# jaehyuck0103/OpenMAVIS

Hardware: AMD Instinct MI355X
Metric: multi-cam frames/sec (ORB extract+match) + LocalBA iters/sec, 5x720x540 (higher is better)
Workload: dtype u8

## Files before the change

### include/omv.h

```cpp
#ifndef OMV_H
#define OMV_H

#include <stddef.h>
#include <stdint.h>

#ifdef __cplusplus
extern "C" {
#endif

typedef int omv_status;
#define OMV_OK 0
#define OMV_ERR_ARG 1
#define OMV_ERR_HIP 2
#define OMV_ERR_CAPACITY 3
#define OMV_ERR_NO_DEVICE 4

typedef struct omv_orb_params {
    int nfeatures;
    float scale_factor;
    int nlevels;
    int ini_th_fast;
    int min_th_fast;
} omv_orb_params;

// ... 38 lines not shown
    float min_x, max_x;
    float min_y, max_y;
    int nlevels;
    float scale_factors[16];
    int cam_model[8];
} omv_frame_geom;

typedef struct omv_mp_view {
    const uint8_t *desc;
    const float *proj_x;
    const float *proj_y;
    const float *view_cos;
    const int32_t *level;
    const uint8_t *in_view;
    const float *track_depth;
    const uint8_t *is_bad;
    const uint8_t *has_obs;
} omv_mp_view;

typedef struct omv_matcher omv_matcher;

omv_status omv_matcher_create(int max_frames, int n_cams, int kp_cap, int max_mps, omv_matcher **out);
omv_status omv_matcher_destroy(omv_matcher *m);

omv_status omv_matcher_assign_grid(omv_matcher *m, int n_frames, const omv_frame_geom *geom, const omv_kp *kps,
                                   const int *n_kp, void *stream);
omv_status omv_matcher_grid_debug(omv_matcher *m, int frame, int cam, int32_t *cell_start, int32_t *idx);

omv_status omv_matcher_search_projection(omv_matcher *m, int n_frames, const omv_frame_geom *geom, const omv_kp *kps,
                                         const uint8_t *desc, const int *n_kp, const omv_mp_view *mps, int M, float th,
                                         int far_points, float th_far, float nnratio, const int32_t *l2r,
                                         const int32_t *r2l, const uint8_t *kp_occ_init, int32_t *kp_to_mp,
                                         int *n_matches, void *stream);

omv_status omv_matcher_stereo_lapping(omv_matcher *m, int n_frames, const uint8_t *desc, const int *n_kp,
                                      const int *mono, double ratio, int32_t *l2r, int32_t *r2l, void *stream);

omv_status omv_matcher_stereo_triangulate(omv_matcher *m, int n_frames, int n_cams, int kp_cap, const omv_kp *kps,
                                          const int *n_kp, const int *mono, const float *cams, const float *Rlr,
                                          const float *tlr, const float *level_sigma2, int nlevels, int32_t *l2r,
                                          int32_t *r2l, float *depth, float *p3d, void *stream);

omv_status omv_matcher_last_error(omv_matcher *m);

omv_status omv_matcher_enable_timing(omv_matcher *m, int on);
omv_status omv_matcher_stage_ms(omv_matcher *m, double *ms4, int reset);

omv_status omv_bf_knn2(int n_pairs, const uint8_t *query, int q_cap, const int *nq, const uint8_t *train, int t_cap,
                       const int *nt, int32_t *idx2, int32_t *dist2, void *stream);
int omv_bf_knn2_path(int n_pairs, int q_cap, int t_cap);

typedef struct omv_se3f {
    float q[4];
    float t[3];
} omv_se3f;

typedef struct omv_last_frame {
    const float *pos;
    const uint8_t *desc;
    const uint8_t *valid;
    const uint8_t *has_obs;
    const omv_kp *kps;
    int S;
} omv_last_frame;

omv_status omv_matcher_search_last_frame(omv_matcher *m, int n_frames, const omv_frame_geom *geom, const omv_kp *kps,
// ... 600 lines not shown
```

### openmavis_amd/_lib.py

```python
import ctypes
import os

_HERE = os.path.dirname(os.path.abspath(__file__))
LIB_PATH = os.path.join(_HERE, "libomv_hip.so")

OMV_OK = 0
OMV_ERR_ARG = 1
OMV_ERR_HIP = 2
OMV_ERR_CAPACITY = 3
OMV_ERR_NO_DEVICE = 4
CAM_KB8 = 0
CAM_PINHOLE = 1
_ERRS = {1: "bad argument", 2: "HIP runtime error", 3: "device capacity exceeded", 4: "no HIP device"}


class OmvError(RuntimeError):
    pass


def check(status, what="omv call"):
    if status != OMV_OK:
        raise OmvError(f"{what} failed: {_ERRS.get(status, status)} ({status})")


# ... 202 lines not shown
                ("trials", ctypes.c_int), ("lambda_", ctypes.c_double), ("lambda_init", ctypes.c_double),
                ("mono_chi2", ctypes.c_void_p), ("mono_outlier", ctypes.c_void_p),
                ("stereo_chi2", ctypes.c_void_p), ("stereo_outlier", ctypes.c_void_p)]


try:
    import numpy as _np

    KP_DTYPE = _np.dtype([("x", "<f4"), ("y", "<f4"), ("size", "<f4"), ("angle", "<f4"),
                          ("response", "<f4"), ("octave", "<i4")])
except ImportError:
    KP_DTYPE = None

_VP, _I, _F, _SZ = ctypes.c_void_p, ctypes.c_int, ctypes.c_float, ctypes.c_size_t
ALLREDUCE_FN = ctypes.CFUNCTYPE(ctypes.c_int, ctypes.c_void_p, ctypes.c_void_p, ctypes.c_size_t, ctypes.c_void_p)
SIGNATURES = {
    "omv_orb_create": (_I, [ctypes.POINTER(OrbParams), _I, _I, _I, ctypes.POINTER(_VP)]),
    "omv_orb_destroy": (_I, [_VP]),
    "omv_selftest_node_sort": (_I, [_VP, _VP, _I, _VP, _VP]),
    "omv_orb_max_keypoints": (_I, [_VP]),
    "omv_orb_scale_tables": (_I, [_VP, _VP, _VP, _VP, _VP]),
    "omv_orb_extract_batch": (_I, [_VP, _I, _VP, _SZ, _SZ, _VP, _VP, _VP, _VP, _VP, _VP]),
    "omv_orb_extract_host": (_I, [_VP, _VP, _SZ, _I, _I, _VP, _VP, _VP, _VP]),
    "omv_orb_last_error": (_I, [_VP]),
    "omv_orb_enable_timing": (_I, [_VP, _I]),
    "omv_orb_set_harris": (_I, [_VP, _VP]),
    "omv_orb_stage_ms": (_I, [_VP, _VP, ctypes.POINTER(ctypes.c_longlong), _I]),
    "omv_orb_last_counts": (_I, [_VP, ctypes.POINTER(ctypes.c_longlong), ctypes.POINTER(ctypes.c_longlong)]),
    "omv_orb_debug_level": (_I, [_VP, _I, _I, _VP, ctypes.POINTER(_I), ctypes.POINTER(_I)]),
    "omv_matcher_create": (_I, [_I, _I, _I, _I, ctypes.POINTER(_VP)]),
    "omv_matcher_destroy": (_I, [_VP]),
    "omv_matcher_assign_grid": (_I, [_VP, _I, ctypes.POINTER(FrameGeom), _VP, _VP, _VP]),
    "omv_matcher_grid_debug": (_I, [_VP, _I, _I, _VP, _VP]),
    "omv_matcher_enable_timing": (_I, [_VP, _I]),
    "omv_matcher_last_error": (_I, [_VP]),
    "omv_matcher_stage_ms": (_I, [_VP, _VP, _I]),
    "omv_matcher_search_projection": (_I, [_VP, _I, ctypes.POINTER(FrameGeom), _VP, _VP, _VP,
                                           ctypes.POINTER(MpView), _I, _F, _I, _F, _F, _VP, _VP, _VP, _VP,
                                           _VP, _VP]),
    "omv_matcher_stereo_lapping": (_I, [_VP, _I, _VP, _VP, _VP, ctypes.c_double, _VP, _VP, _VP]),
    "omv_bf_knn2": (_I, [_I, _VP, _I, _VP, _VP, _I, _VP, _VP, _VP, _VP]),
    "omv_bf_knn2_path": (_I, [_I, _I, _I]),
    "omv_matcher_search_last_frame": (_I, [_VP, _I, ctypes.POINTER(FrameGeom), _VP, _VP, _VP, _VP, _VP, _VP,
                                           ctypes.POINTER(SE3f), ctypes.POINTER(LastFrame), _F, _I, _F, _I, _VP, _VP,
                                           _VP, _VP]),
    "omv_frustum": (_I, [_I, _VP, ctypes.POINTER(Rig), ctypes.POINTER(MpWorld), _I, _F, ctypes.POINTER(MpTrack), _VP,
                         _VP]),
    "omv_lba_create": (_I, [_I, _I, _I, _I, _I, ctypes.POINTER(_VP)]),
    "omv_lba_destroy": (_I, [_VP]),
    "omv_lba_set_problem": (_I, [_VP, ctypes.POINTER(LbaProblem)]),
    "omv_lba_optimize": (_I, [_VP, ctypes.POINTER(LbaOpts), ctypes.POINTER(LbaProblem), ctypes.POINTER(LbaResult)]),
    "omv_lba_evaluate": (_I, [_VP, _VP, _VP, _VP, _VP]),
    "omv_lba_evaluate_stereo": (_I, [_VP, _VP, _VP, _VP]),
    "omv_lba_stage_ms": (_I, [_VP, _VP, ctypes.POINTER(_I)]),
    "omv_lba_host_syncs": (_I, [_VP, ctypes.POINTER(_I), ctypes.POINTER(_I)]),
    "omv_lba_enable_timing": (_I, [_VP, _I]),
    "omv_lba_set_driver": (_I, [_VP, _I]),
    "omv_lba_reset": (_I, [_VP]),
    "omv_lba_set_comm": (_I, [_VP, _I, _I, _VP, _VP]),
    "omv_tri_debug": (_I, [_VP, _VP, _VP, _VP, _VP, _VP, _F, _F, _VP]),
    "omv_matcher_stereo_triangulate": (_I, [_VP, _I, _I, _I, _VP, _VP, _VP, _VP, _VP, _VP, _VP, _I, _VP, _VP, _VP,
                                            _VP, _VP]),
    "omv_matcher_search_for_triangulation": (_I, [_VP, _I, ctypes.POINTER(TriPair), _VP, _VP, _I, _I, _I, _VP, _VP]),
    "omv_matcher_search_by_bow": (_I, [_VP, _I, ctypes.POINTER(BowJob), _I, _F, _I, _VP, _VP]),
    "omv_matcher_bow_rescans": (_I, [ctypes.POINTER(ctypes.c_int64), _I]),
    "omv_matcher_search_for_initialization": (_I, [_VP, _I, _VP, ctypes.POINTER(FrameGeom), _VP, _VP, _VP, _VP, _I,
# ... 124 lines not shown
```

### openmavis_amd/csrc/match.hip

```cpp
#include <hip/hip_runtime.h>

#include <climits>
#include <cstdlib>
#include <cstring>
#include <type_traits>
#include <cmath>
#include <cstdio>
#include <vector>

#include "../../include/omv.h"
#include "omv_camera.h"
#include "omv_device.h"
#include "omv_host.h"

namespace {

using omv::kGridCols, omv::kGridRows;
constexpr int kCells = omv::kGridCells;
constexpr int kTH_HIGH = 100;
constexpr int kTop = 16;
constexpr int kMaxCams = 8;
constexpr size_t kResolveLds = 150 * 1024;

struct FrameArgs {
// ... 140 lines not shown
    int count;
    __device__ __forceinline__ void reset() { key[0] = key[1] = ~0ull, count = 0; }
    __device__ __forceinline__ void insert_at(int idx, int dist, int oct, int q) {
        const uint64_t k = ((uint64_t)dist << 40) | ((uint64_t)q << 20) | ((uint64_t)oct << 16) | (uint64_t)idx;
        key[1] = k < key[0] ? key[0] : (k < key[1] ? k : key[1]);
        key[0] = k < key[0] ? k : key[0];
    }
};
__device__ __forceinline__ uint32_t key_rec(uint64_t k) {
    return (uint32_t)(k & 0xffff) | ((uint32_t)(k >> 40) << 16) | ((uint32_t)((k >> 16) & 0xf) << 25);
}

struct TopSeq {
    uint32_t key[kTop];
    int n, count;
    __device__ __forceinline__ void reset() {
#pragma unroll
        for (int q = 0; q < kTop; ++q) key[q] = ~0u;
        n = count = 0;
    }
    __device__ __forceinline__ void insert(int idx, int dist, int oct) {
        const uint32_t k = ((uint32_t)dist << 23) | ((uint32_t)oct << 16) | (uint32_t)idx;
        const uint32_t kk = k | 0x7fffffu;
#pragma unroll
        for (int q = kTop - 1; q > 0; --q) key[q] = kk < key[q - 1] ? key[q - 1] : (kk < key[q] ? k : key[q]);
        key[0] = kk < key[0] ? k : key[0];
        n = min(n + 1, kTop);
    }
    __device__ __forceinline__ int idx(int q) const { return (int)(key[q] & 0xffff); }
    __device__ __forceinline__ int oct(int q) const { return (int)((key[q] >> 16) & 0x7f); }
    __device__ __forceinline__ int dist(int q) const { return (int)(key[q] >> 23); }
    __device__ __forceinline__ uint32_t rec(int q) const {
        return (uint32_t)idx(q) | ((uint32_t)dist(q) << 16) | ((uint32_t)oct(q) << 25);
    }
};

template <class Blocked, class TopT>
__device__ void scan_window(const FrameArgs &f, int frame, int cam, float x, float y, float r, int minL, int maxL,
                            const uint64_t dmp[4], Blocked blocked, TopT &t) {
    t.reset();
    omv::GridRange w;
    OMV_GRID_WINDOW_OR(x, y, r, f.min_x, f.min_y, f.invW, f.invH, w, return)
    const bool checkLevels = (minL > 0) || (maxL >= 0);
    const size_t fc = (size_t)frame * f.n_cams + cam;
    const int32_t *cs = f.cell_start + fc * (kCells + 1);
    const int32_t *ci = f.cell_idx + fc * f.kp_cap;
    const omv_kp *kp = f.kps + fc * f.kp_cap;
    const uint8_t *dd = f.desc + fc * f.kp_cap * 32;
    for (int ix = w.x0; ix <= w.x1; ++ix) {
        const int c0 = ix * kGridRows + w.y0, c1 = ix * kGridRows + w.y1;
        const int e = cs[c1 + 1];
        int p = cs[c0];
        int inext = p < e ? ci[p] : 0;
        for (; p < e; ++p) {
            const int i = inext;
            if (p + 1 < e) inext = ci[p + 1];
            const omv_kp k = kp[i];
            uint64_t d[4];
            omv::load_desc(dd + (size_t)i * 32, d);
            if (checkLevels) {
                if (k.octave < minL) continue;
                if (maxL >= 0 && k.octave > maxL) continue;
            }
            if (!(fabsf(k.x - x) < r && fabsf(k.y - y) < r)) continue;
            if (blocked(cam * f.kp_cap + i)) continue;
            ++t.count;
// ... 135 lines not shown
    const int g = lane % G;
    for (int q0 = 0; q0 < nq; q0 += 64 / G) {
        if (q0 + lane / G >= nq) break;
        const long long gid = g0 + queue[wave][q0 + lane / G];
        const int c = (int)(gid % C);
        const long long fm = gid / C;
        const int frame = (int)(fm / m.M);
        const size_t bc = (size_t)gid;
        std::conditional_t<G == 1, TopSeq, Top> t;
        t.reset();
        uint64_t dmp[4];
        omv::load_desc(m.desc + (size_t)fm * 32, dmp);
        const float r = window_radius(f, m, bc, c, th, th != 1.0f);
        const uint8_t *occ = occ_init ? occ_init + (size_t)frame * C * f.kp_cap : nullptr;
        if constexpr (G == 1) {
            scan_window(f, frame, c, m.proj_x[bc], m.proj_y[bc], r, m.level[bc] - 1, m.level[bc], dmp,
                        [&](int slot) { return occ && occ[slot]; }, t);
        } else {
            scan_window_coop<G>(f, frame, c, m.proj_x[bc], m.proj_y[bc], r, m.level[bc] - 1, m.level[bc], dmp,
                                [&](int slot) { return occ && occ[slot]; }, t, g);
            merge_top<G>(t);
        }
        if (g == 0) store_record(&recs[bc], t);
    }
}

constexpr int kStageThreads = 512;
constexpr uint32_t kStageBlocked = 1u << 31;
constexpr size_t kStageLdsMax = 80 * 1024;
constexpr int kScanGroup = 4;
constexpr int kStageUnroll = 3;
constexpr int kStageMaxIt = 4;
constexpr int kStageBuckets = 32;

__host__ __device__ inline size_t stage_lds_bytes(int kp_cap, int pw) {
    return (size_t)kp_cap * (32 + 8 + 4) + (size_t)(kCells + 1) * 4 + (size_t)(kStageThreads / 64) * pw * 4;
}

__device__ __forceinline__ void scan_window_lds(const FrameArgs &f, float x, float y, float r, int minL, int maxL,
                                                const uint64_t dmp[4], const int *scs, const float2 *sxy,
                                                const uint32_t *smeta, const uint4 *sdesc, TopSeq &t) {
    t.reset();
    omv::GridRange w;
    OMV_GRID_WINDOW_OR(x, y, r, f.min_x, f.min_y, f.invW, f.invH, w, return)
    const bool checkLevels = (minL > 0) || (maxL >= 0);
    for (int ix = w.x0; ix <= w.x1; ++ix) {
        const int e = scs[ix * kGridRows + w.y1 + 1];
        for (int p0 = scs[ix * kGridRows + w.y0]; p0 < e; p0 += kScanGroup) {
            float2 k[kScanGroup];
            uint32_t meta[kScanGroup];
#pragma unroll
            for (int u = 0; u < kScanGroup; ++u) k[u] = sxy[p0 + u], meta[u] = smeta[p0 + u];
#pragma unroll
            for (int u = 0; u < kScanGroup; ++u) {
                const int oct = (int)((meta[u] >> 16) & 0x7f);
                bool ok = p0 + u < e;
                if (checkLevels) ok = ok && oct >= minL && !(maxL >= 0 && oct > maxL);
                ok = ok && fabsf(k[u].x - x) < r && fabsf(k[u].y - y) < r && !(meta[u] & kStageBlocked);
                if (!ok) continue;
                const int p = p0 + u;
                const uint4 a = sdesc[2 * p], b = sdesc[2 * p + 1];
                const uint64_t d[4] = {(uint64_t)a.x | ((uint64_t)a.y << 32), (uint64_t)a.z | ((uint64_t)a.w << 32),
                                       (uint64_t)b.x | ((uint64_t)b.y << 32), (uint64_t)b.z | ((uint64_t)b.w << 32)};
                ++t.count;
                t.insert((int)(meta[u] & 0xffff), omv::hamming256(dmp, d), oct);
            }
        }
    }
}

__global__ void __launch_bounds__(kStageThreads) cand_stage_kernel(FrameArgs f, MpArgs m, int n_frames, float th,
                                                                   const uint8_t *occ_init, Rec *recs, int *counts,
                                                                   int *flags, int far_points, float th_far,
                                                                   int n_chunks, int pw, int n_blocks) {
    extern __shared__ __align__(16) unsigned char stage_lds[];
    const int C = f.n_cams, cap = f.kp_cap, M = m.M;
    const int blk = omv::xcd_block(n_blocks);
    if (blk < 0) return;
    const int chunk = blk % n_chunks, fc = blk / n_chunks, cam = fc % C, frame = fc / C;
    uint4 *sdesc = reinterpret_cast<uint4 *>(stage_lds);
    float2 *sxy = reinterpret_cast<float2 *>(stage_lds + (size_t)cap * 32);
    uint32_t *smeta = reinterpret_cast<uint32_t *>(stage_lds + (size_t)cap * 40);
    int *scs = reinterpret_cast<int *>(stage_lds + (size_t)cap * 44);
    int *queue = scs + kCells + 1;
    __shared__ int bucket[kStageBuckets + 1];
    const int tid = threadIdx.x, wave = tid >> 6, lane = tid & 63;
    if (tid <= kStageBuckets) bucket[tid] = 0;
    __syncthreads();
    const int32_t *cs = f.cell_start + (size_t)fc * (kCells + 1);
    const int32_t *ci = f.cell_idx + (size_t)fc * cap;
    const omv_kp *kp = f.kps + (size_t)fc * cap;
    const uint4 *dd = reinterpret_cast<const uint4 *>(f.desc + (size_t)fc * cap * 32);
    const uint8_t *occ = occ_init ? occ_init + ((size_t)frame * C + cam) * cap : nullptr;
    const int n_in = cs[kCells];
    for (int c = tid; c <= kCells; c += kStageThreads) scs[c] = cs[c];
    int idx[kStageUnroll];
#pragma unroll
    for (int u = 0; u < kStageUnroll; ++u) {
        const int p = u * kStageThreads + tid;
        idx[u] = p < n_in ? ci[p] : -1;
    }
    const int p0 = chunk * (kStageThreads / 64) * pw;
    int key[kStageMaxIt], lv[kStageMaxIt];
    bool iv[kStageMaxIt];
    float vc[kStageMaxIt];
#pragma unroll
    for (int it = 0; it < kStageMaxIt; ++it) {
        const int i = p0 + wave * pw + it * 64 + lane;
        const bool valid = it * 64 + lane < pw && i < M;
        const size_t bc = ((size_t)frame * M + (valid ? i : 0)) * C + cam;
        iv[it] = valid && m.in_view[bc];
        lv[it] = valid ? m.level[bc] : -1;
        vc[it] = valid ? m.view_cos[bc] : 0.0f;
    }
#pragma unroll
    for (int it = 0; it < kStageMaxIt; ++it) {
        key[it] = -1;
        const int i = p0 + wave * pw + it * 64 + lane;
        if (it * 64 + lane >= pw || i >= M) continue;
        const size_t fm = (size_t)frame * M + i, bc = fm * C + cam;
        if (cam == 0) {
            flags[fm] = point_flags(m, f, fm, frame, i, C, far_points, th_far);
        }
        if (iv[it] && lv[it] >= 0 && lv[it] < f.nlevels) {
            key[it] = 2 * lv[it] + (vc[it] > 0.998 ? 0 : 1);
            atomicAdd(&bucket[key[it]], 1);
        }
    }
    for (int s0 = 0; s0 < n_in; s0 += kStageThreads * kStageUnroll) {
        if (s0 > 0) {
#pragma unroll
            for (int u = 0; u < kStageUnroll; ++u) {
                const int p = s0 + u * kStageThreads + tid;
                idx[u] = p < n_in ? ci[p] : -1;
            }
        }
        float x[kStageUnroll], y[kStageUnroll];
        int oct[kStageUnroll];
        uint4 da[kStageUnroll], db[kStageUnroll];
        bool bl[kStageUnroll];
#pragma unroll
        for (int u = 0; u < kStageUnroll; ++u) {
            const int i = max(idx[u], 0);
            x[u] = kp[i].x, y[u] = kp[i].y, oct[u] = kp[i].octave;
            da[u] = dd[2 * i], db[u] = dd[2 * i + 1];
            bl[u] = occ && occ[i];
        }
#pragma unroll
        for (int u = 0; u < kStageUnroll; ++u) {
            const int p = s0 + u * kStageThreads + tid;
            if (idx[u] < 0) continue;
            sxy[p] = make_float2(x[u], y[u]);
            smeta[p] = (uint32_t)idx[u] | ((uint32_t)(oct[u] & 0x7f) << 16) | (bl[u] ? kStageBlocked : 0u);
            sdesc[2 * p] = da[u], sdesc[2 * p + 1] = db[u];
        }
    }
    __syncthreads();
    if (tid < 64) {
        const int c = tid < kStageBuckets ? bucket[tid] : 0;
        const int incl = omv::wave_incl_scan_i32(c, lane);
        if (tid < kStageBuckets) bucket[tid] = incl - c;
        if (tid == kStageBuckets - 1) bucket[kStageBuckets] = incl;
    }
    __syncthreads();
#pragma unroll
    for (int it = 0; it < kStageMaxIt; ++it)
        if (key[it] >= 0) queue[atomicAdd(&bucket[key[it]], 1)] = wave * pw + it * 64 + lane;
    __syncthreads();
    const int nq = bucket[kStageBuckets];
    for (int q = wave * 64 + lane; q - lane < nq; q += kStageThreads) {
        if (q >= nq) break;
        const int i = p0 + queue[q];
        const size_t fm = (size_t)frame * M + i, bc = fm * C + cam;
        TopSeq t;
        uint64_t dmp[4];
        omv::load_desc(m.desc + fm * 32, dmp);
        const float r = window_radius(f, m, bc, cam, th, th != 1.0f);
        scan_window_lds(f, m.proj_x[bc], m.proj_y[bc], r, m.level[bc] - 1, m.level[bc], dmp, scs, sxy, smeta, sdesc, t);
        store_record(&recs[bc], t);
    }
}

constexpr int kMaxRevived = 64;
constexpr int kMaxDomains = kMaxCams - 1;
constexpr int kListCap = 128;

struct ResolveArgs {
    FrameArgs f;
    MpArgs m;
    const Rec *recs;
    const int *counts;
    const int *flags;
    const int32_t *l2r, *r2l;
    const uint8_t *occ_init;
    int32_t *kp_to_mp;
    int *n_matches;
    int *err;
    float th, th_far, nnratio;
    int far_points;
    int lds_k2m;
};


__device__ __forceinline__ bool bit_of(const uint32_t *bits, int s) { return (bits[s >> 5] >> (s & 31)) & 1u; }

__device__ bool in_window(const FrameArgs &f, int frame, int c, int slot, float x, float y, float r, int lvl) {
    const omv_kp k = f.kps[((size_t)frame * f.n_cams) * f.kp_cap + slot];
    const int px = (int)roundf((k.x - f.min_x) * f.invW), py = (int)roundf((k.y - f.min_y) * f.invH);
    if (px < 0 || px >= kGridCols || py < 0 || py >= kGridRows) return false;
    const int x0 = max(0, (int)floorf((x - f.min_x - r) * f.invW));
    const int x1 = min(kGridCols - 1, (int)ceilf((x - f.min_x + r) * f.invW));
    const int y0 = max(0, (int)floorf((y - f.min_y - r) * f.invH));
    const int y1 = min(kGridRows - 1, (int)ceilf((y - f.min_y + r) * f.invH));
// ... 1572 lines not shown
omv_status omv_frustum(int n_frames, const omv_frame_pose *poses, const omv_rig *rig, const omv_mp_world *mp, int M,
                       float viewing_cos_limit, const omv_mp_track *out, int32_t *n_in_view, void *stream) {
    if (n_frames <= 0 || !poses || !rig || !mp || !out || M < 0 || rig->n_cams <= 0 || rig->n_cams > kMaxCams ||
        rig->n_levels <= 0 || !cam_models_ok(rig->model, rig->n_cams))
        return OMV_ERR_ARG;
    if (M == 0) return OMV_OK;
    hipStream_t st = (hipStream_t)stream;
    frustum_kernel<<<dim3((M + 255) / 256, n_frames), 256, 0, st>>>(poses, *rig, *mp, M, viewing_cos_limit, *out,
                                                                    n_in_view);
    HIP_OK(hipGetLastError());
    return OMV_OK;
}

omv_status omv_matcher_create(int max_frames, int n_cams, int kp_cap, int max_mps, omv_matcher **out) {
    if (!out || max_frames <= 0 || n_cams <= 0 || n_cams > kMaxCams || kp_cap <= 0 || kp_cap > 65535 || max_mps < 0)
        return OMV_ERR_ARG;
    if (resolve_lds_bytes(n_cams, kp_cap, max_mps) > kResolveLds - kResolveStaticLds || lf_resolve_lds_bytes(n_cams, kp_cap) > kResolveLds)
        return OMV_ERR_ARG;
    int ndev = 0;
    if (hipGetDeviceCount(&ndev) != hipSuccess || ndev == 0) return OMV_ERR_NO_DEVICE;
    const int resolve_dyn = (int)(kResolveLds - kResolveStaticLds);
    HIP_OK(hipFuncSetAttribute((const void *)resolve_kernel<true>, hipFuncAttributeMaxDynamicSharedMemorySize, resolve_dyn));
    HIP_OK(hipFuncSetAttribute((const void *)resolve_kernel<false>, hipFuncAttributeMaxDynamicSharedMemorySize, resolve_dyn));
    HIP_OK(hipFuncSetAttribute((const void *)lf_resolve_kernel, hipFuncAttributeMaxDynamicSharedMemorySize, (int)kResolveLds));
    HIP_OK(hipFuncSetAttribute((const void *)cand_stage_kernel, hipFuncAttributeMaxDynamicSharedMemorySize, (int)kStageLdsMax));
    auto h = std::make_unique<omv_matcher>();
    h->max_frames = max_frames, h->n_cams = n_cams, h->kp_cap = kp_cap, h->max_mps = max_mps;
    if (const char *e = getenv("OMV_BOW_TOP")) h->knobs.bow_top = atoi(e);
    if (const char *e = getenv("OMV_TRI_SLICES")) h->knobs.tri_slices = atoi(e);
    if (const char *e = getenv("OMV_TRI_ECAP")) h->knobs.tri_ecap = atoi(e);
    if (const char *e = getenv("OMV_TRI_WALK")) h->knobs.tri_walk_seq = strcmp(e, "seq") == 0 ? 1 : 0;
    if (const char *e = getenv("OMV_CAND")) h->knobs.cand_mode = strcmp(e, "global") == 0 ? 1 : strcmp(e, "lds") == 0 ? 2 : 0;
    if (const char *e = getenv("OMV_CAND_PW")) h->knobs.cand_pw = atoi(e);
    h->knobs.knn_mode = knn_mode_env(), h->knobs.knn_idx_limit = knn_idx_limit_env();
    const size_t fc = (size_t)max_frames * n_cams;
    const size_t knn = (size_t)2 * max_frames * kp_cap;
    omv::DeviceArena &mem = h->mem;
    if (!mem.alloc(&h->d_cell_start, fc * (kCells + 1)) || !mem.alloc(&h->d_cell_idx, fc * kp_cap) ||
        !mem.alloc(&h->d_recs, fc * max_mps) || !mem.alloc(&h->d_counts, fc * max_mps) ||
        !mem.alloc(&h->d_flags, (size_t)max_frames * max_mps) || !mem.alloc(&h->d_knn_i, knn) ||
        !mem.alloc(&h->d_knn_d, knn) || !mem.alloc(&h->d_err, 1))
        return OMV_ERR_HIP;
    HIP_OK(hipMemset(h->d_err, 0, sizeof(int)));
    *out = h.release();
    return OMV_OK;
}

omv_status omv_matcher_enable_timing(omv_matcher *h, int on) {
    if (!h) return OMV_ERR_ARG;
    h->timing = on != 0;
    return OMV_OK;
}

omv_status omv_matcher_stage_ms(omv_matcher *h, double *ms4, int reset) {
    if (!h || !ms4) return OMV_ERR_ARG;
    HIP_OK(hipStreamSynchronize(h->last));
    for (auto &p : h->ev) {
        float ms = 0.f;
        (void)hipEventElapsedTime(&ms, p.second.first, p.second.second);
        h->stage_ms[p.first] += ms;
        (void)hipEventDestroy(p.second.first);
        (void)hipEventDestroy(p.second.second);
    }
    h->ev.clear();
    for (int k = 0; k < 4; ++k) ms4[k] = h->stage_ms[k];
    if (reset)
// ... 9 lines not shown
    HIP_OK(hipMemset(h->d_err, 0, sizeof(int)));
    return e;
}

omv_status omv_matcher_destroy(omv_matcher *h) {
    if (!h) return OMV_ERR_ARG;
    delete h;
    return OMV_OK;
}

omv_status omv_matcher_assign_grid(omv_matcher *h, int n_frames, const omv_frame_geom *g, const omv_kp *kps,
                                   const int *n_kp, void *stream) {
    if (!h || !g || !kps || !n_kp || n_frames <= 0 || n_frames > h->max_frames || g->n_cams != h->n_cams)
        return OMV_ERR_ARG;
    FrameArgs f;
    if (!cam_models_ok(g->cam_model, h->n_cams)) return OMV_ERR_ARG;
    fill_frame(h, g, kps, nullptr, n_kp, f);
    hipStream_t st = (hipStream_t)stream;
    h->last = st;
    hipEvent_t e0 = h->timing ? mk_event(st) : nullptr;
    grid_kernel<<<n_frames * h->n_cams, 256, 0, st>>>(f, h->d_cell_start, h->d_cell_idx);
    if (h->timing) h->ev.push_back({0, {e0, mk_event(st)}});
    HIP_OK(hipGetLastError());
    return OMV_OK;
}

omv_status omv_matcher_grid_debug(omv_matcher *h, int frame, int cam, int32_t *cell_start, int32_t *idx) {
    if (!h || frame < 0 || frame >= h->max_frames || cam < 0 || cam >= h->n_cams) return OMV_ERR_ARG;
    HIP_OK(hipStreamSynchronize(h->last));
    const size_t fc = (size_t)frame * h->n_cams + cam;
    HIP_OK(hipMemcpy(cell_start, h->d_cell_start + fc * (kCells + 1), sizeof(int32_t) * (kCells + 1),
                     hipMemcpyDeviceToHost));
    HIP_OK(hipMemcpy(idx, h->d_cell_idx + fc * h->kp_cap, sizeof(int32_t) * h->kp_cap, hipMemcpyDeviceToHost));
    return OMV_OK;
}

omv_status omv_matcher_search_projection(omv_matcher *h, int n_frames, const omv_frame_geom *g, const omv_kp *kps,
                                         const uint8_t *desc, const int *n_kp, const omv_mp_view *mps, int M, float th,
                                         int far_points, float th_far, float nnratio, const int32_t *l2r,
                                         const int32_t *r2l, const uint8_t *kp_occ_init, int32_t *kp_to_mp,
                                         int *n_matches, void *stream) {
    if (!h || !g || !kps || !desc || !n_kp || !mps || !kp_to_mp || !n_matches || n_frames <= 0 ||
        n_frames > h->max_frames || M < 0 || M > h->max_mps || g->n_cams != h->n_cams)
        return OMV_ERR_ARG;
    if (h->n_cams > 1 && (!l2r || !r2l)) return OMV_ERR_ARG;
    hipStream_t st = (hipStream_t)stream;
    h->last = st;
    FrameArgs f;
    if (!cam_models_ok(g->cam_model, h->n_cams)) return OMV_ERR_ARG;
    fill_frame(h, g, kps, desc, n_kp, f);
    MpArgs m{mps->desc, mps->proj_x, mps->proj_y, mps->view_cos, mps->level, mps->in_view, mps->track_depth,
             mps->is_bad, mps->has_obs, M};
    hipEvent_t e0 = h->timing ? mk_event(st) : nullptr;
    if (M > 0) {
        const long long tot = (long long)n_frames * M * h->n_cams;
        int pw = 128;
        while (pw > 16 && (long long)n_frames * h->n_cams * ((M + 8 * pw - 1) / (8 * pw)) < 1024) pw >>= 1;
        if (h->knobs.cand_pw > 0) pw = min(h->knobs.cand_pw, 64 * kStageMaxIt);
        const bool staged = h->knobs.cand_mode == 2 || (h->knobs.cand_mode == 0 && tot > 262144);
        if (staged && stage_lds_bytes(h->kp_cap, pw) <= kStageLdsMax) {
            const int n_chunks = (M + 8 * pw - 1) / (8 * pw);
            const int nb = n_frames * h->n_cams * n_chunks;
            cand_stage_kernel<<<omv::xcd_grid(nb), kStageThreads, stage_lds_bytes(h->kp_cap, pw), st>>>(
                f, m, n_frames, th, kp_occ_init, h->d_recs, h->d_counts, h->d_flags, far_points, th_far, n_chunks, pw, nb);
        } else if (tot <= 65536) {
            const int nb = (int)((tot + 4 * (kCandChunk / 16) - 1) / (4 * (kCandChunk / 16)));
            cand_kernel<16><<<omv::xcd_grid(nb), 256, 0, st>>>(f, m, n_frames, th, kp_occ_init, h->d_recs, h->d_counts,
                                                               h->d_flags, far_points, th_far, nb);
        } else if (tot <= 262144) {
            const int nb = (int)((tot + 4 * (kCandChunk / 8) - 1) / (4 * (kCandChunk / 8)));
            cand_kernel<8><<<omv::xcd_grid(nb), 256, 0, st>>>(f, m, n_frames, th, kp_occ_init, h->d_recs, h->d_counts,
                                                              h->d_flags, far_points, th_far, nb);
        } else {
            const int nb = (int)((tot + 4 * kCandChunk - 1) / (4 * kCandChunk));
            cand_kernel<1><<<omv::xcd_grid(nb), 256, 0, st>>>(f, m, n_frames, th, kp_occ_init, h->d_recs, h->d_counts,
                                                              h->d_flags, far_points, th_far, nb);
        }
    }
    hipEvent_t e1 = h->timing ? mk_event(st) : nullptr;
    hipEvent_t e2 = h->timing ? mk_event(st) : nullptr;
    int staged = 1;
    const size_t lds = resolve_lds_bytes(h->n_cams, h->kp_cap, M, &staged);
    ResolveArgs ra{f, m, h->d_recs, h->d_counts, h->d_flags, l2r, r2l, kp_occ_init, kp_to_mp, n_matches, h->d_err, th, th_far, nnratio,
                   far_points, staged};
    const int n_dom = 1 + max(0, h->n_cams - 2);
    if (staged)
        resolve_kernel<true><<<n_frames, 64 * n_dom, lds, st>>>(ra);
    else
        resolve_kernel<false><<<n_frames, 64 * n_dom, lds, st>>>(ra);
    if (h->timing) {
        h->ev.push_back({2, {e0, e1}});
        h->ev.push_back({3, {e2, mk_event(st)}});
    }
    HIP_OK(hipGetLastError());
    return OMV_OK;
}

// ... 216 lines not shown
```

### openmavis_amd/csrc/omv_device.h

```cpp
#pragma once
#include <hip/hip_runtime.h>
#include <stdint.h>

#include "omv_math.h"

namespace omv {


__device__ __forceinline__ int reflect101(int p, int n) {
    p = p < 0 ? -p : p;
    return p >= n ? 2 * n - 2 - p : p;
}

__device__ __forceinline__ int hamming256(const uint64_t *a, const uint64_t *b) {
    return __popcll(a[0] ^ b[0]) + __popcll(a[1] ^ b[1]) + __popcll(a[2] ^ b[2]) + __popcll(a[3] ^ b[3]);
}
__device__ __forceinline__ void load_desc(const uint8_t *p, uint64_t d[4]) {
    const uint64_t *q = reinterpret_cast<const uint64_t *>(p);
    d[0] = q[0], d[1] = q[1], d[2] = q[2], d[3] = q[3];
}

__device__ __forceinline__ void wave_lds_sync() {
    __builtin_amdgcn_fence(__ATOMIC_RELEASE, "wavefront");
    __builtin_amdgcn_wave_barrier();
// ... 22 lines not shown
        const int t = __shfl_up(v, d, 64);
        if (lane >= d) v += t;
    }
    return v;
}

__device__ __forceinline__ double rcp_nr(double x) {
    double r = __builtin_amdgcn_rcp(x);
    double e = __builtin_fma(-x, r, 1.0);
    r = __builtin_fma(r, e, r);
    e = __builtin_fma(-x, r, 1.0);
    return __builtin_fma(r, e, r);
}


__device__ __forceinline__ int xcd_block(int n_logical) {
    const int chunk = (n_logical + 7) >> 3;
    const int b = (int)(blockIdx.x & 7) * chunk + (int)(blockIdx.x >> 3);
    return b < n_logical ? b : -1;
}
__host__ inline int xcd_grid(int n_logical) { return (n_logical + 7) & ~7; }

}
extern "C" __device__ __attribute__((const)) uint32_t omv_llvm_mul_u24(uint32_t, uint32_t) __asm("llvm.amdgcn.mul.u24.i32");
extern "C" __device__ __attribute__((const)) uint32_t omv_llvm_mulhi_u24(uint32_t, uint32_t) __asm("llvm.amdgcn.mulhi.u24");
namespace omv {
__device__ __forceinline__ int mul_u24(int a, int b) { return (int)omv_llvm_mul_u24((uint32_t)a, (uint32_t)b); }
__device__ __forceinline__ uint32_t mulhi_u24(uint32_t a, uint32_t b) { return omv_llvm_mulhi_u24(a, b); }

struct MatcherKnobs {
    int bow_top = -1, tri_slices = -1, tri_ecap = -1, tri_walk_seq = 0;
    int cand_mode = 0;
    int cand_pw = -1;
    int knn_mode = 0;
    int knn_idx_limit = 1 << 16;
};
MatcherKnobs matcher_knobs(const struct ::omv_matcher *m);
size_t matcher_kf_entry_cap(const struct ::omv_matcher *m);

}
```

### openmavis_amd/matcher.py

```python
import ctypes

import numpy as np

from . import _lib

FRAME_GRID_COLS = 64
FRAME_GRID_ROWS = 48
TH_HIGH = 100
TH_LOW = 50
HISTO_LENGTH = 30


def frame_geom(n_cams, width, height, scale_factors, cam_model=None):
    g = _lib.FrameGeom()
    g.n_cams = n_cams
    g.min_x, g.max_x, g.min_y, g.max_y = 0.0, float(width), 0.0, float(height)
    g.nlevels = len(scale_factors)
    for i, s in enumerate(scale_factors):
        g.scale_factors[i] = float(s)
    for i, m in enumerate(cam_model if cam_model is not None else ()):
        g.cam_model[i] = {"kb8": _lib.CAM_KB8, "pinhole": _lib.CAM_PINHOLE}.get(m, m) if isinstance(m, str) else int(m)
    return g


# ... 103 lines not shown
        try:
            self.close()
        except Exception:
            pass

    @staticmethod
    def _stream(stream):
        return ctypes.c_void_p(stream.cuda_stream) if stream is not None else None

    def AssignFeaturesToGrid(self, frames, stream=None):
        h = self._handle(frames)
        _lib.check(self._lib.omv_matcher_assign_grid(h, frames.n_frames, ctypes.byref(frames.geom),
                                                     _lib.ptr(frames.kps), _lib.ptr(frames.n_kp),
                                                     self._stream(stream)), "omv_matcher_assign_grid")

    STAGES = ("grid", "stereo_knn", "proj_candidates", "proj_resolve")

    def enable_timing(self, on=True):
        _lib.check(self._lib.omv_matcher_enable_timing(self._h, int(bool(on))))

    def stage_ms(self, reset=True):
        ms = np.zeros(4, np.float64)
        _lib.check(self._lib.omv_matcher_stage_ms(self._h, _lib.ptr(ms), int(bool(reset))))
        return dict(zip(self.STAGES, ms.tolist()))

    def last_error(self):
        return self._lib.omv_matcher_last_error(self._h)

    def grid(self, frame, cam):
        cs = np.zeros(FRAME_GRID_COLS * FRAME_GRID_ROWS + 1, np.int32)
        idx = np.zeros(self._shape[2], np.int32)
        _lib.check(self._lib.omv_matcher_grid_debug(self._h, frame, cam, _lib.ptr(cs), _lib.ptr(idx)))
        return cs, idx[:cs[-1]]

    def SearchByProjectionLastFrame(self, frames, last, Tcw, Tlw, cams, Trl, th, bMono=False, mb=0.0, stream=None):
        h = self._handle(frames, last["pos"].shape[1])
        self.AssignFeaturesToGrid(frames, stream)
        S = last["pos"].shape[1]
        lf = _lib.LastFrame(_lib.ptr(last["pos"]), _lib.ptr(last["desc"]), _lib.ptr(last["valid"]),
                            _lib.ptr(last["has_obs"]), _lib.ptr(last["kps"]), S)
        c = np.ascontiguousarray(np.asarray(cams, np.float32).reshape(-1, 8)[:frames.n_cams])
        trl = _lib.SE3f()
        t7 = np.asarray(Trl, np.float32).reshape(7)
        for q in range(4):
            trl.q[q] = float(t7[q])
        for q in range(3):
            trl.t[q] = float(t7[4 + q])
        _lib.check(self._lib.omv_matcher_search_last_frame(
            h, frames.n_frames, ctypes.byref(frames.geom), _lib.ptr(frames.kps), _lib.ptr(frames.desc),
            _lib.ptr(frames.n_kp), _lib.ptr(c), _lib.ptr(Tcw), _lib.ptr(Tlw), ctypes.byref(trl), ctypes.byref(lf),
            ctypes.c_float(th), int(bool(bMono)), ctypes.c_float(mb), int(self.mbCheckOrientation),
            _lib.ptr(frames.occ_init), _lib.ptr(frames.kp_to_mp), _lib.ptr(frames.n_matches), self._stream(stream)),
            "omv_matcher_search_last_frame")
        return frames.n_matches

    def StereoTriangulate(self, frames, cams, Rlr, tlr, level_sigma2, stream=None):
        import torch
        if not hasattr(frames, "depth"):
            frames.depth = torch.full((frames.n_frames, frames.kp_cap), -1.0, dtype=torch.float32,
                                      device=frames.l2r.device)
            frames.p3d = torch.zeros((frames.n_frames, frames.kp_cap, 3), dtype=torch.float32, device=frames.l2r.device)
        h = self._handle(frames)
        c = np.ascontiguousarray(np.asarray(cams, np.float32).reshape(-1, 8)[:2])
        R = np.ascontiguousarray(np.asarray(Rlr, np.float32).reshape(9))
        t = np.ascontiguousarray(np.asarray(tlr, np.float32).reshape(3))
        sg = np.ascontiguousarray(np.asarray(level_sigma2, np.float32))
# ... 240 lines not shown
```

Baseline: 51720.

## Load-balance projection candidate scan by splitting heavy windows across cooperating lanes

The LDS candidate-stage kernel now bins map points by the number of grid entries their search window covers. Points with large windows are processed by groups of 2 to 64 lanes that scan strided subsets, keep a per-lane top-K by position, and merge through shuffle-based bitonic merges. Waves take work items from a shared atomic task counter instead of a fixed assignment, which is meant to remove wave imbalance from a few expensive windows. This adds a second grid-window pass, more buckets, merge overhead and register pressure, plus a records debug API and an optional profiling printf.

```diff
diff --git a/include/omv.h b/include/omv.h
--- a/include/omv.h
+++ b/include/omv.h
@@ -94,6 +94,7 @@
                                          int far_points, float th_far, float nnratio, const int32_t *l2r,
                                          const int32_t *r2l, const uint8_t *kp_occ_init, int32_t *kp_to_mp,
                                          int *n_matches, void *stream);
+omv_status omv_matcher_records_debug(omv_matcher *m, int n_frames, int M, uint32_t *out);
 
 omv_status omv_matcher_stereo_lapping(omv_matcher *m, int n_frames, const uint8_t *desc, const int *n_kp,
                                       const int *mono, double ratio, int32_t *l2r, int32_t *r2l, void *stream);
diff --git a/openmavis_amd/_lib.py b/openmavis_amd/_lib.py
--- a/openmavis_amd/_lib.py
+++ b/openmavis_amd/_lib.py
@@ -258,6 +258,7 @@
     "omv_matcher_destroy": (_I, [_VP]),
     "omv_matcher_assign_grid": (_I, [_VP, _I, ctypes.POINTER(FrameGeom), _VP, _VP, _VP]),
     "omv_matcher_grid_debug": (_I, [_VP, _I, _I, _VP, _VP]),
+    "omv_matcher_records_debug": (_I, [_VP, _I, _I, _VP]),
     "omv_matcher_enable_timing": (_I, [_VP, _I]),
     "omv_matcher_last_error": (_I, [_VP]),
     "omv_matcher_stage_ms": (_I, [_VP, _VP, _I]),
diff --git a/openmavis_amd/csrc/match.hip b/openmavis_amd/csrc/match.hip
--- a/openmavis_amd/csrc/match.hip
+++ b/openmavis_amd/csrc/match.hip
@@ -196,6 +196,41 @@
     __device__ __forceinline__ int dist(int q) const { return (int)(key[q] >> 23); }
     __device__ __forceinline__ uint32_t rec(int q) const {
         return (uint32_t)idx(q) | ((uint32_t)dist(q) << 16) | ((uint32_t)oct(q) << 25);
+    }
+};
+
+struct TopPos {
+    uint32_t key[kTop];
+    int count;
+    __device__ __forceinline__ void reset() {
+#pragma unroll
+        for (int q = 0; q < kTop; ++q) key[q] = ~0u;
+        count = 0;
+    }
+    __device__ __forceinline__ void insert(int p, int dist) {
+        const uint32_t k = ((uint32_t)dist << 16) | (uint32_t)p;
+#pragma unroll
+        for (int q = kTop - 1; q > 0; --q) key[q] = k < key[q - 1] ? key[q - 1] : min(k, key[q]);
+        key[0] = min(k, key[0]);
+    }
+    __device__ __forceinline__ void merge(int G) {
+        for (int s = 1; s < G; s <<= 1) {
+            uint32_t o[kTop];
+#pragma unroll
+            for (int q = 0; q < kTop; ++q) o[q] = (uint32_t)__shfl_xor((int)key[q], s, 64);
+            count += __shfl_xor(count, s, 64);
+#pragma unroll
+            for (int q = 0; q < kTop; ++q) key[q] = min(key[q], o[kTop - 1 - q]);
+#pragma unroll
+            for (int d = kTop / 2; d > 0; d >>= 1) {
+#pragma unroll
+                for (int q = 0; q < kTop; ++q) {
+                    if (q & d) continue;
+                    const uint32_t lo = min(key[q], key[q + d]), hi = max(key[q], key[q + d]);
+                    key[q] = lo, key[q + d] = hi;
+                }
+            }
+        }
     }
 };
 
@@ -397,9 +432,51 @@
 constexpr int kStageUnroll = 3;
 constexpr int kStageMaxIt = 4;
 constexpr int kStageBuckets = 32;
+constexpr int kStageClasses = 7;
+constexpr int kStageKeys = kStageClasses * kStageBuckets;
+constexpr int kStageSplit = 64;
 
 __host__ __device__ inline size_t stage_lds_bytes(int kp_cap, int pw) {
     return (size_t)kp_cap * (32 + 8 + 4) + (size_t)(kCells + 1) * 4 + (size_t)(kStageThreads / 64) * pw * 4;
+}
+
+template <class Ins>
+__device__ __forceinline__ int scan_run_lds(int pb, int sh, int cnt, float x, float y, float r, bool checkLevels,
+                                            int minL, int maxL, const uint64_t dmp[4], const float2 *sxy,
+                                            const uint32_t *smeta, const uint4 *sdesc, Ins ins) {
+    int found = 0;
+    for (int k0 = 0; k0 < cnt; k0 += 32) {
+        const int nk = min(32, cnt - k0);
+        uint32_t mask = 0;
+        for (int u0 = 0; u0 < nk; u0 += kScanGroup) {
+            float2 k[kScanGroup];
+            uint32_t meta[kScanGroup];
+#pragma unroll
+            for (int u = 0; u < kScanGroup; ++u) {
+                const int p = pb + ((u0 + u < nk ? k0 + u0 + u : k0) << sh);
+                k[u] = sxy[p], meta[u] = smeta[p];
+            }
+#pragma unroll
+            for (int u = 0; u < kScanGroup; ++u) {
+                const int oct = (int)((meta[u] >> 16) & 0x7f);
+                bool ok = u0 + u < nk;
+                if (checkLevels) ok = ok && oct >= minL && !(maxL >= 0 && oct > maxL);
+                ok = ok && fabsf(k[u].x - x) < r && fabsf(k[u].y - y) < r && !(meta[u] & kStageBlocked);
+                mask |= (uint32_t)ok << (u0 + u);
+            }
+        }
+        found += __popc(mask);
+        while (mask) {
+            const int p = pb + ((k0 + __ffs((int)mask) - 1) << sh);
+            mask &= mask - 1;
+            const uint32_t meta = smeta[p];
+            const uint4 a = sdesc[2 * p], b = sdesc[2 * p + 1];
+            const uint64_t d[4] = {(uint64_t)a.x | ((uint64_t)a.y << 32), (uint64_t)a.z | ((uint64_t)a.w << 32),
+                                   (uint64_t)b.x | ((uint64_t)b.y << 32), (uint64_t)b.z | ((uint64_t)b.w << 32)};
+            ins(p, meta, omv::hamming256(dmp, d));
+        }
+    }
+    return found;
 }
 
 __device__ __forceinline__ void scan_window_lds(const FrameArgs &f, float x, float y, float r, int minL, int maxL,
@@ -410,34 +487,49 @@
     OMV_GRID_WINDOW_OR(x, y, r, f.min_x, f.min_y, f.invW, f.invH, w, return)
     const bool checkLevels = (minL > 0) || (maxL >= 0);
     for (int ix = w.x0; ix <= w.x1; ++ix) {
-        const int e = scs[ix * kGridRows + w.y1 + 1];
-        for (int p0 = scs[ix * kGridRows + w.y0]; p0 < e; p0 += kScanGroup) {
-            float2 k[kScanGroup];
-            uint32_t meta[kScanGroup];
-#pragma unroll
-            for (int u = 0; u < kScanGroup; ++u) k[u] = sxy[p0 + u], meta[u] = smeta[p0 + u];
-#pragma unroll
-            for (int u = 0; u < kScanGroup; ++u) {
-                const int oct = (int)((meta[u] >> 16) & 0x7f);
-                bool ok = p0 + u < e;
-                if (checkLevels) ok = ok && oct >= minL && !(maxL >= 0 && oct > maxL);
-                ok = ok && fabsf(k[u].x - x) < r && fabsf(k[u].y - y) < r && !(meta[u] & kStageBlocked);
-                if (!ok) continue;
-                const int p = p0 + u;
-                const uint4 a = sdesc[2 * p], b = sdesc[2 * p + 1];
-                const uint64_t d[4] = {(uint64_t)a.x | ((uint64_t)a.y << 32), (uint64_t)a.z | ((uint64_t)a.w << 32),
-                                       (uint64_t)b.x | ((uint64_t)b.y << 32), (uint64_t)b.z | ((uint64_t)b.w << 32)};
-                ++t.count;
-                t.insert((int)(meta[u] & 0xffff), omv::hamming256(dmp, d), oct);
-            }
-        }
-    }
+        const int b = scs[ix * kGridRows + w.y0], e = scs[ix * kGridRows + w.y1 + 1];
+        t.count += scan_run_lds(b, 0, e - b, x, y, r, checkLevels, minL, maxL, dmp, sxy, smeta, sdesc,
+                                [&](int, uint32_t meta, int dist) {
+                                    t.insert((int)(meta & 0xffff), dist, (int)((meta >> 16) & 0x7f));
+                                });
+    }
+}
+
+__device__ __forceinline__ void scan_window_lds_coop(const omv::GridRange &w, float x, float y, float r, int minL, int maxL,
+                                                     const uint64_t dmp[4], const int *scs, const float2 *sxy,
+                                                     const uint32_t *smeta, const uint4 *sdesc, TopPos &t, int g, int sh) {
+    const bool checkLevels = (minL > 0) || (maxL >= 0);
+    int pos = g, acc = 0;
+    for (int ix = w.x0; ix <= w.x1; ++ix) {
+        const int b = scs[ix * kGridRows + w.y0], end = acc + scs[ix * kGridRows + w.y1 + 1] - b;
+        if (pos < end) {
+            const int cnt = (end - pos + (1 << sh) - 1) >> sh;
+            t.count += scan_run_lds(b + pos - acc, sh, cnt, x, y, r, checkLevels, minL, maxL, dmp, sxy, smeta, sdesc,
+                                    [&](int p, uint32_t, int dist) { t.insert(p, dist); });
+            pos += cnt << sh;
+        }
+        acc = end;
+    }
+}
+
+__device__ __forceinline__ void store_record_pos(Rec *dst, const TopPos &t, const uint32_t *smeta) {
+    uint4 *o4 = reinterpret_cast<uint4 *>(dst);
+    uint32_t w[kTop];
+#pragma unroll
+    for (int q = 0; q < kTop; ++q) {
+        const uint32_t k = t.key[q];
+        const uint32_t meta = smeta[k == ~0u ? 0u : (k & 0xffffu)];
+        w[q] = k == ~0u ? 0u : ((meta & 0xffffu) | ((k >> 16) << 16) | (((meta >> 16) & 0x7fu) << 25) | kRecValid);
+    }
+    w[0] |= t.count > kTop ? kRecOver : 0u;
+#pragma unroll
+    for (int v = 0; v < kTop / 4; ++v) o4[v] = make_uint4(w[4 * v], w[4 * v + 1], w[4 * v + 2], w[4 * v + 3]);
 }
 
 __global__ void __launch_bounds__(kStageThreads) cand_stage_kernel(FrameArgs f, MpArgs m, int n_frames, float th,
                                                                    const uint8_t *occ_init, Rec *recs, int *counts,
                                                                    int *flags, int far_points, float th_far,
-                                                                   int n_chunks, int pw, int n_blocks) {
+                                                                   int n_chunks, int pw, int n_blocks, int split) {
     extern __shared__ __align__(16) unsigned char stage_lds[];
     const int C = f.n_cams, cap = f.kp_cap, M = m.M;
     const int blk = omv::xcd_block(n_blocks);
@@ -448,16 +540,22 @@
     uint32_t *smeta = reinterpret_cast<uint32_t *>(stage_lds + (size_t)cap * 40);
     int *scs = reinterpret_cast<int *>(stage_lds + (size_t)cap * 44);
     int *queue = scs + kCells + 1;
-    __shared__ int bucket[kStageBuckets + 1];
+    __shared__ int bucket[kStageKeys + 1];
+    __shared__ int next_task;
     const int tid = threadIdx.x, wave = tid >> 6, lane = tid & 63;
-    if (tid <= kStageBuckets) bucket[tid] = 0;
+    if (tid <= kStageKeys) bucket[tid] = 0;
+    if (tid == 0) next_task = 0;
     __syncthreads();
     const int32_t *cs = f.cell_start + (size_t)fc * (kCells + 1);
     const int32_t *ci = f.cell_idx + (size_t)fc * cap;
     const omv_kp *kp = f.kps + (size_t)fc * cap;
     const uint4 *dd = reinterpret_cast<const uint4 *>(f.desc + (size_t)fc * cap * 32);
     const uint8_t *occ = occ_init ? occ_init + ((size_t)frame * C + cam) * cap : nullptr;
+#ifdef OMV_STAGE_PROFILE
+    long long tp[4] = {wall_clock64(), 0, 0, 0};
+#endif
     const int n_in = cs[kCells];
+    const bool balance = split < n_in;
     for (int c = tid; c <= kCells; c += kStageThreads) scs[c] = cs[c];
     int idx[kStageUnroll];
 #pragma unroll
@@ -468,7 +566,7 @@
     const int p0 = chunk * (kStageThreads / 64) * pw;
     int key[kStageMaxIt], lv[kStageMaxIt];
     bool iv[kStageMaxIt];
-    float vc[kStageMaxIt];
+    float vc[kStageMaxIt], px[kStageMaxIt], py[kStageMaxIt];
 #pragma unroll
     for (int it = 0; it < kStageMaxIt; ++it) {
         const int i = p0 + wave * pw + it * 64 + lane;
@@ -477,6 +575,7 @@
         iv[it] = valid && m.in_view[bc];
         lv[it] = valid ? m.level[bc] : -1;
         vc[it] = valid ? m.view_cos[bc] : 0.0f;
+        px[it] = m.proj_x[bc], py[it] = m.proj_y[bc];
     }
 #pragma unroll
     for (int it = 0; it < kStageMaxIt; ++it) {
@@ -489,7 +588,7 @@
         }
         if (iv[it] && lv[it] >= 0 && lv[it] < f.nlevels) {
             key[it] = 2 * lv[it] + (vc[it] > 0.998 ? 0 : 1);
-            atomicAdd(&bucket[key[it]], 1);
+            if (!balance) atomicAdd(&bucket[key[it]], 1);
         }
     }
     for (int s0 = 0; s0 < n_in; s0 += kStageThreads * kStageUnroll) {
@@ -521,29 +620,95 @@
         }
     }
     __syncthreads();
+#ifdef OMV_STAGE_PROFILE
+    tp[1] = wall_clock64();
+#endif
+    if (balance) {
+#pragma unroll
+        for (int it = 0; it < kStageMaxIt; ++it) {
+            if (key[it] < 0) continue;
+            float r = vc[it] > 0.998 ? 2.5f : 4.0f;
+            if (cam == 0 && th != 1.0f) r *= th;
+            r *= f.scale[lv[it]];
+            omv::GridRange w;
+            int entries = 0;
+            if (omv::grid_window(px[it], py[it], r, f.min_x, f.min_y, f.invW, f.invH, w))
+                for (int ix = w.x0; ix <= w.x1; ++ix) entries += scs[ix * kGridRows + w.y1 + 1] - scs[ix * kGridRows + w.y0];
+            int cls = 0;
+#pragma unroll
+            for (int k = 0; k < kStageClasses - 1; ++k) cls += entries > (split << k);
+            key[it] += cls * kStageBuckets;
+            atomicAdd(&bucket[key[it]], 1);
+        }
+        __syncthreads();
+    }
     if (tid < 64) {
-        const int c = tid < kStageBuckets ? bucket[tid] : 0;
-        const int incl = omv::wave_incl_scan_i32(c, lane);
-        if (tid < kStageBuckets) bucket[tid] = incl - c;
-        if (tid == kStageBuckets - 1) bucket[kStageBuckets] = incl;
+        int c[4], s = 0;
+#pragma unroll
+        for (int k = 0; k < 4; ++k) c[k] = 4 * tid + k < kStageKeys ? bucket[4 * tid + k] : 0, s += c[k];
+        int run = omv::wave_incl_scan_i32(s, lane) - s;
+#pragma unroll
+        for (int k = 0; k < 4; ++k) {
+            if (4 * tid + k < kStageKeys) bucket[4 * tid + k] = run;
+            run += c[k];
+        }
+        if (tid == 63) bucket[kStageKeys] = run;
     }
     __syncthreads();
 #pragma unroll
     for (int it = 0; it < kStageMaxIt; ++it)
         if (key[it] >= 0) queue[atomicAdd(&bucket[key[it]], 1)] = wave * pw + it * 64 + lane;
     __syncthreads();
-    const int nq = bucket[kStageBuckets];
-    for (int q = wave * 64 + lane; q - lane < nq; q += kStageThreads) {
-        if (q >= nq) break;
+#ifdef OMV_STAGE_PROFILE
+    tp[2] = wall_clock64();
+#endif
+    int cend[kStageClasses];
+#pragma unroll
+    for (int k = 0; k < kStageClasses; ++k)
+        cend[k] = __builtin_amdgcn_readfirstlane(bucket[k * kStageBuckets + kStageBuckets - 1]);
+    for (;;) {
+        int rem = 0;
+        if (lane == 0) rem = atomicAdd(&next_task, 1);
+        rem = __builtin_amdgcn_readfirstlane(rem);
+        int cls = -1, q0 = 0, q1 = 0;
+#pragma unroll
+        for (int k = kStageClasses - 1; k >= 0; --k) {
+            const int st = k ? cend[k - 1] : 0, sh = 6 - k, nt = (cend[k] - st + (1 << sh) - 1) >> sh;
+            if (cls < 0 && rem < nt) cls = k, q1 = cend[k] - (rem << sh), q0 = max(st, q1 - (1 << sh));
+            if (cls < 0) rem -= nt;
+        }
+        if (cls < 0) break;
+        const int G = 1 << cls, q = q0 + (lane >> cls);
+        if (q >= q1) continue;
         const int i = p0 + queue[q];
         const size_t fm = (size_t)frame * M + i, bc = fm * C + cam;
-        TopSeq t;
         uint64_t dmp[4];
         omv::load_desc(m.desc + fm * 32, dmp);
         const float r = window_radius(f, m, bc, cam, th, th != 1.0f);
-        scan_window_lds(f, m.proj_x[bc], m.proj_y[bc], r, m.level[bc] - 1, m.level[bc], dmp, scs, sxy, smeta, sdesc, t);
-        store_record(&recs[bc], t);
-    }
+        const float x = m.proj_x[bc], y = m.proj_y[bc];
+        const int lvl = m.level[bc];
+        if (cls == 0) {
+            TopSeq t;
+            scan_window_lds(f, x, y, r, lvl - 1, lvl, dmp, scs, sxy, smeta, sdesc, t);
+            store_record(&recs[bc], t);
+        } else {
+            TopPos t;
+            t.reset();
+            omv::GridRange w;
+            if (omv::grid_window(x, y, r, f.min_x, f.min_y, f.invW, f.invH, w))
+                scan_window_lds_coop(w, x, y, r, lvl - 1, lvl, dmp, scs, sxy, smeta, sdesc, t, lane & (G - 1), cls);
+            t.merge(G);
+            if ((lane & (G - 1)) == 0) store_record_pos(&recs[bc], t, smeta);
+        }
+    }
+#ifdef OMV_STAGE_PROFILE
+    tp[3] = wall_clock64();
+    __syncthreads();
+    if (lane == 0 && frame == 1 && chunk <= 1)
+        printf("cand_stage cam %d chunk %d wave %d slots %d of them split %d ticks(100MHz): stage %lld sort %lld scan %lld wait %lld\n",
+               cam, chunk, wave, cend[kStageClasses - 1], cend[kStageClasses - 1] - cend[0], tp[1] - tp[0], tp[2] - tp[1],
+               tp[3] - tp[2], wall_clock64() - tp[3]);
+#endif
 }
 
 constexpr int kMaxRevived = 64;
@@ -2182,6 +2347,7 @@
     if (const char *e = getenv("OMV_TRI_WALK")) h->knobs.tri_walk_seq = strcmp(e, "seq") == 0 ? 1 : 0;
     if (const char *e = getenv("OMV_CAND")) h->knobs.cand_mode = strcmp(e, "global") == 0 ? 1 : strcmp(e, "lds") == 0 ? 2 : 0;
     if (const char *e = getenv("OMV_CAND_PW")) h->knobs.cand_pw = atoi(e);
+    if (const char *e = getenv("OMV_CAND_SPLIT")) h->knobs.cand_split = (int)std::min<long long>(atoll(e), (1 << 24) - 1);
     h->knobs.knn_mode = knn_mode_env(), h->knobs.knn_idx_limit = knn_idx_limit_env();
     const size_t fc = (size_t)max_frames * n_cams;
     const size_t knn = (size_t)2 * max_frames * kp_cap;
@@ -2257,6 +2423,13 @@
     HIP_OK(hipMemcpy(cell_start, h->d_cell_start + fc * (kCells + 1), sizeof(int32_t) * (kCells + 1),
                      hipMemcpyDeviceToHost));
     HIP_OK(hipMemcpy(idx, h->d_cell_idx + fc * h->kp_cap, sizeof(int32_t) * h->kp_cap, hipMemcpyDeviceToHost));
+    return OMV_OK;
+}
+
+omv_status omv_matcher_records_debug(omv_matcher *h, int n_frames, int M, uint32_t *out) {
+    if (!h || !out || n_frames <= 0 || n_frames > h->max_frames || M <= 0 || M > h->max_mps) return OMV_ERR_ARG;
+    HIP_OK(hipStreamSynchronize(h->last));
+    HIP_OK(hipMemcpy(out, h->d_recs, sizeof(Rec) * n_frames * M * h->n_cams, hipMemcpyDeviceToHost));
     return OMV_OK;
 }
 
@@ -2287,7 +2460,8 @@
             const int n_chunks = (M + 8 * pw - 1) / (8 * pw);
             const int nb = n_frames * h->n_cams * n_chunks;
             cand_stage_kernel<<<omv::xcd_grid(nb), kStageThreads, stage_lds_bytes(h->kp_cap, pw), st>>>(
-                f, m, n_frames, th, kp_occ_init, h->d_recs, h->d_counts, h->d_flags, far_points, th_far, n_chunks, pw, nb);
+                f, m, n_frames, th, kp_occ_init, h->d_recs, h->d_counts, h->d_flags, far_points, th_far, n_chunks, pw, nb,
+                h->knobs.cand_split > 0 ? h->knobs.cand_split : kStageSplit);
         } else if (tot <= 65536) {
             const int nb = (int)((tot + 4 * (kCandChunk / 16) - 1) / (4 * (kCandChunk / 16)));
             cand_kernel<16><<<omv::xcd_grid(nb), 256, 0, st>>>(f, m, n_frames, th, kp_occ_init, h->d_recs, h->d_counts,
diff --git a/openmavis_amd/csrc/omv_device.h b/openmavis_amd/csrc/omv_device.h
--- a/openmavis_amd/csrc/omv_device.h
+++ b/openmavis_amd/csrc/omv_device.h
@@ -78,6 +78,7 @@
     int bow_top = -1, tri_slices = -1, tri_ecap = -1, tri_walk_seq = 0;
     int cand_mode = 0;
     int cand_pw = -1;
+    int cand_split = -1;
     int knn_mode = 0;
     int knn_idx_limit = 1 << 16;
 };
diff --git a/openmavis_amd/matcher.py b/openmavis_amd/matcher.py
--- a/openmavis_amd/matcher.py
+++ b/openmavis_amd/matcher.py
@@ -159,6 +159,11 @@
         idx = np.zeros(self._shape[2], np.int32)
         _lib.check(self._lib.omv_matcher_grid_debug(self._h, frame, cam, _lib.ptr(cs), _lib.ptr(idx)))
         return cs, idx[:cs[-1]]
+
+    def records(self, n_frames, M):
+        out = np.zeros((n_frames, M, self._shape[1], 16), np.uint32)
+        _lib.check(self._lib.omv_matcher_records_debug(self._h, n_frames, M, _lib.ptr(out)))
+        return out
 
     def SearchByProjectionLastFrame(self, frames, last, Tcw, Tlw, cams, Trl, th, bMono=False, mb=0.0, stream=None):
         h = self._handle(frames, last["pos"].shape[1])
```

Result: faster. 52580 (median of 6 runs) (+1.7%).
